# smhassanerfani/nasa-niswan

Hardware: AMD Instinct MI355X
Metric: training samples/sec (90x144x20 grid, seq_len=12) (higher is better)
Workload: dtype bf16; 1 GPU; cfg1-20level; in_channels=62, out_channels=20, seq_len=12, batch_per_gpu=8, global_batch=8, parallelism=dp1, wave=4, overlap_allreduce=False

## Files before the change

nasa-niswan_amd/csrc/wgrad.hip:

```cpp
#include <type_traits>
#include "nint_common.h"

struct WgSrc {
  const char* dG;
  const char* src; long src_img_stride; int src_pix_stride;
  float* partial;
  int CB, JG;
  int nblk;
  int ntiles, tiles_per_split;
  int want_db;
};
struct WgradArgs {
  long dG_img_stride; int dG_pix_stride;
  WgSrc s[2];
  int nparts;
  int NTC, J;
  int TG;
  int k, p, taps;
  int P, Wh;
  int tiles_x, tiles_y;
};

template <int DT> struct WgTile;
template <> struct WgTile<NINT_BF16> { static constexpr int PR = 4, RA = 160; static constexpr int rb(int ntc) { return ntc == 1 ? 32 : 96; } };
template <> struct WgTile<NINT_F32> { static constexpr int PR = 2, RA = 320; static constexpr int rb(int ntc) { return ntc == 1 ? 64 : 192; } };

template <int DT, int JW, int NS, int KS, int NTCT, int KX>
__global__ __launch_bounds__(256, 2) void wgrad_kernel(WgradArgs a) {
  typedef Elem<DT> E;
  typedef WgTile<DT> TT;
  constexpr int PR = TT::PR, RA = TT::RA;
  constexpr int NTN = 4 / NS;
  constexpr int A_UNITS_PIX = 64 * E::ES / 16;

  extern __shared__ __attribute__((aligned(16))) char smem[];
  const int tid = threadIdx.x, lane = tid & 63;
  const int wave = __builtin_amdgcn_readfirstlane(tid >> 6);
  constexpr int p = KS / 2, k = KS;
  constexpr int HWt = 32 + 2 * p, HHt = PR + 2 * p;
  constexpr int RB = TT::rb(NTCT);
  constexpr int b_units_pix = 16 * NTCT * E::ES / 16;
  constexpr int UA_ROW = RA / 16, NA_U = PR * 32 * UA_ROW;
  constexpr int UB_PIX = RB / 16, NB_U = HHt * HWt * UB_PIX, NB_U_PAD = (NB_U + 63) / 64 * 64;
  constexpr int a_bytes = PR * 32 * RA;
  constexpr int b_bytes = NB_U_PAD * 16;
  constexpr int buf_bytes = a_bytes + b_bytes;
  static_assert(NA_U % 64 == 0 && a_bytes % 1024 == 0, "whole DMA pieces");
  constexpr int NI_A = NA_U / 64, NI_B = NB_U_PAD / 64, NI = NI_A + NI_B;

  int by = blockIdx.y, part = 0;
  if (a.nparts == 2) {
    const int per_nb = a.s[0].CB + a.s[1].CB;
    const int nbq = by / per_nb, r = by - nbq * per_nb;
    part = r >= a.s[0].CB ? 1 : 0;
    by = part ? nbq * a.s[1].CB + (r - a.s[0].CB) : nbq * a.s[0].CB + r;
  }
  part = __builtin_amdgcn_readfirstlane(part);
  by = __builtin_amdgcn_readfirstlane(by);
  struct { const char* dG; const char* src; long src_img_stride; int src_pix_stride; float* partial; int CB, JG, nblk, ntiles, tiles_per_split, want_db; } S;
  {
    const WgSrc& T = a.s[part];
    S.dG = T.dG; S.src = T.src; S.src_img_stride = T.src_img_stride; S.src_pix_stride = T.src_pix_stride; S.partial = T.partial;
    S.CB = T.CB; S.JG = T.JG; S.nblk = T.nblk; S.ntiles = T.ntiles; S.tiles_per_split = T.tiles_per_split; S.want_db = T.want_db;
  }
  const int tg = __builtin_amdgcn_readfirstlane(by % a.TG);
  const int bc = __builtin_amdgcn_readfirstlane(by / a.TG);
  const int nb = bc / S.CB, cb = bc % S.CB;
  const int jb = tg * 4 * JW;
  const int t_begin = blockIdx.x * S.tiles_per_split;
  const int t_end = min(S.ntiles, t_begin + S.tiles_per_split);
  const int i0 = (wave % NS) * NTN;
  const int j0 = (wave / NS) * JW;

  f32x4_t acc[NTN][JW];
#pragma unroll
  for (int i = 0; i < NTN; ++i)
#pragma unroll
    for (int j = 0; j < JW; ++j) acc[i][j] = (f32x4_t){0.f, 0.f, 0.f, 0.f};

  const bool do_db = __builtin_amdgcn_readfirstlane((S.want_db && cb == 0 && tg == a.TG - 1 && wave == 3 && NS == 1) ? 1 : 0);

  constexpr int NI_WM = (NI + 1) / 2;
  int p_begin, p_cnt;
  {
    constexpr int CM = (DT == NINT_BF16 ? 16 : 32 * 4) * NTN * PR, CD = 100;
    int nv[4], n16[4], tot = 0, sum_nv = 0;
#pragma unroll
    for (int w = 0; w < 4; ++w) { nv[w] = min(JW, max(0, a.J - jb - (w / NS) * JW)); sum_nv += nv[w]; }
    const int L = (NI * CD + CM * sum_nv) / 4;
#pragma unroll
    for (int w = 0; w < 4; ++w) { n16[w] = max(0, (L - nv[w] * CM) * 16 / CD); tot += n16[w]; }
    int cnt[4], prev = 0, acc16 = 0, excess = 0;
#pragma unroll
    for (int w = 0; w < 4; ++w) {
      acc16 += n16[w];
      const int e = w == 3 ? NI : (tot > 0 ? min(NI, (acc16 * NI + tot / 2) / tot) : (w + 1) * NI / 4);
      cnt[w] = e - prev;
      prev = e;
      if (cnt[w] > NI_WM) { excess += cnt[w] - NI_WM; cnt[w] = NI_WM; }
    }
#pragma unroll
    for (int w = 0; w < 4; ++w) {
      const int take = min(NI_WM - cnt[w], excess);
      cnt[w] += take;
      excess -= take;
    }
    const int s1 = cnt[0], s2 = s1 + cnt[1], s3 = s2 + cnt[2];
    p_begin = __builtin_amdgcn_readfirstlane(wave == 0 ? 0 : (wave == 1 ? s1 : (wave == 2 ? s2 : s3)));
    p_cnt = __builtin_amdgcn_readfirstlane(wave == 0 ? cnt[0] : (wave == 1 ? cnt[1] : (wave == 2 ? cnt[2] : cnt[3])));
  }
  unsigned doff[NI_WM];
#pragma unroll
  for (int i = 0; i < NI_WM; ++i) {
    const int t = p_begin + i;
    unsigned o = 0;
    if (t < NI_A) {
      const int u = t * 64 + lane;
      const int pix = u / UA_ROW, q = u - pix * UA_ROW;
      if (q < A_UNITS_PIX) o = (unsigned)(((pix >> 5) * a.Wh + (pix & 31)) * a.dG_pix_stride + q * 16);
    } else if (t < NI) {
      const int u = (t - NI_A) * 64 + lane;
      const int hp = u / UB_PIX, q = u - hp * UB_PIX;
      const int hy = hp / HWt, hx = hp - hy * HWt;
      if (hp < HHt * HWt && q < b_units_pix) o = (unsigned)((hy * a.Wh + hx) * S.src_pix_stride + q * 16);
    }
    doff[i] = o;
  }
  int ld_tx, ld_ty, ld_img;
  {
    const int r = t_begin / a.tiles_x;
    ld_tx = t_begin - r * a.tiles_x;
    ld_img = r / a.tiles_y;
    ld_ty = r - ld_img * a.tiles_y;
  }
  const char* const ga0 = S.dG + nb * 64 * E::ES;
  const char* const gb0 = S.src + cb * 16 * NTCT * E::ES;

  auto issue_dma = [&](char* buf) {
    const int y0 = ld_ty * PR, x0 = ld_tx * 32;
    const char* ga = ga0 + (long)ld_img * a.dG_img_stride + ((long)(y0 + a.P) * a.Wh + (x0 + a.P)) * a.dG_pix_stride;
    const char* gb = gb0 + (long)ld_img * S.src_img_stride + ((long)(y0 + a.P - p) * a.Wh + (x0 + a.P - p)) * S.src_pix_stride;
#pragma unroll
    for (int i = 0; i < NI_WM; ++i) {
      const int t = p_begin + i;
      if (i < p_cnt) {
        const char* src = (t < NI_A ? ga : gb) + doff[i];
        char* dst = buf + (t < NI_A ? t * 1024 : a_bytes + (t - NI_A) * 1024);
        unsigned keep;
        const unsigned lds_dst = __builtin_amdgcn_readfirstlane((unsigned)(uintptr_t)(__attribute__((address_space(3))) char*)dst);
        asm volatile("s_mov_b32 %0, m0\n\ts_mov_b32 m0, %2\n\ts_nop 0\n\tglobal_load_lds_dwordx4 %1, off\n\ts_mov_b32 m0, %0"
                     : "=&s"(keep) : "v"(src), "s"(lds_dst) : "memory");
      }
    }
    const bool wx = ld_tx + 1 == a.tiles_x;
    const bool wy = wx && (ld_ty + 1 == a.tiles_y);
    ld_tx = wx ? 0 : ld_tx + 1;
    ld_ty = wy ? 0 : (wx ? ld_ty + 1 : ld_ty);
    ld_img += wy ? 1 : 0;
  };

  if (t_begin < t_end) issue_dma(smem);
  asm volatile("s_waitcnt vmcnt(0)" ::: "memory");
  __syncthreads();

  const int g = lane >> 4, i16 = lane & 15;
  int vB[JW];
  int vA;
  const int nvalid = __builtin_amdgcn_readfirstlane(min(JW, max(0, a.J - jb - j0)));
  constexpr int JT = KS * KX * NTCT;
  constexpr int XO = KX == KS ? 0 : p;
  constexpr int NVL = JT % JW == 0 ? JW : JT % JW;
  if constexpr (DT == NINT_BF16) {
    const int q = i16 >> 2, p8 = (i16 & 3) * 8;
    vA = (4 * g + q) * RA + i0 * 32 + p8;
#pragma unroll
    for (int jj = 0; jj < JW; ++jj) {
      const int j = min(jb + j0 + jj, a.J - 1);
      const int tap = j / NTCT, ct = j - tap * NTCT;
      const int tyy = tap / KX, txx = tap - tyy * KX + XO;
      vB[jj] = a_bytes + (tyy * HWt + txx + 4 * g + q) * RB + ct * 32 + p8;
    }
  } else {
    vA = g * RA + (i0 * 16 + i16) * 4;
#pragma unroll
    for (int jj = 0; jj < JW; ++jj) {
      const int j = min(jb + j0 + jj, a.J - 1);
      const int tap = j / NTCT, ct = j - tap * NTCT;
      const int tyy = tap / KX, txx = tap - tyy * KX + XO;
      vB[jj] = a_bytes + (tyy * HWt + txx + g) * RB + (ct * 16 + i16) * 4;
    }
  }
  auto run_tiles = [&](auto nvc, auto dbc) __attribute__((always_inline)) {
    constexpr int NV = decltype(nvc)::value;
    constexpr bool DB = decltype(dbc)::value;
    for (int tile = t_begin; tile < t_end; ++tile) {
      const int cur = (tile - t_begin) & 1;
      const bool more = tile + 1 < t_end;
      if (more) issue_dma(smem + (cur ^ 1) * buf_bytes);
      const char* Ab = smem + cur * buf_bytes + vA;
      const char* Bb[JW];
#pragma unroll
      for (int jj = 0; jj < JW; ++jj) Bb[jj] = smem + cur * buf_bytes + vB[jj];
      if constexpr ((NV > 0 || DB) && DT == NINT_BF16) {
#pragma unroll
        for (int pr = 0; pr < PR; ++pr) {
          auto read_tr = [&](const char* ad, int half) __attribute__((always_inline)) {
            s16x4_t lo = __builtin_amdgcn_ds_read_tr16_b64_v4i16((__attribute__((address_space(3))) s16x4_t*)(ad));
            s16x4_t hi = __builtin_amdgcn_ds_read_tr16_b64_v4i16((__attribute__((address_space(3))) s16x4_t*)(ad + half));
            u32x2_t l2 = __builtin_bit_cast(u32x2_t, lo), h2 = __builtin_bit_cast(u32x2_t, hi);
            return (u32x4_t){l2[0], l2[1], h2[0], h2[1]};
          };
          u32x4_t af[NTN], bf[NV > 0 ? NV : 1];
#pragma unroll
          for (int i = 0; i < NTN; ++i) af[i] = read_tr(Ab + pr * 32 * RA + i * 32, 16 * RA);
#pragma unroll
          for (int jj = 0; jj < NV; ++jj) bf[jj] = read_tr(Bb[jj] + pr * HWt * RB, 16 * RB);
#pragma unroll
          for (int jj = 0; jj < NV; ++jj)
#pragma unroll
            for (int i = 0; i < NTN; ++i) acc[i][jj] = mma_step<NINT_BF16>(af[i], bf[jj], acc[i][jj]);
          if constexpr (DB) {
            const u32x4_t ones = {0x3f803f80u, 0x3f803f80u, 0x3f803f80u, 0x3f803f80u};
#pragma unroll
            for (int i = 0; i < NTN; ++i) acc[i][JW - 1] = mma_step<NINT_BF16>(af[i], ones, acc[i][JW - 1]);
          }
        }
      } else if constexpr (NV > 0 || DB) {
#pragma unroll
        for (int pr = 0; pr < PR; ++pr) {
#pragma unroll
          for (int ks = 0; ks < 2; ++ks) {
#pragma unroll
            for (int m = 0; m < 4; ++m) {
              float af[NTN];
#pragma unroll
              for (int i = 0; i < NTN; ++i)
                af[i] = *(const float*)(Ab + (pr * 32 + ks * 16 + 4 * m) * RA + i * 64);
#pragma unroll
              for (int jj = 0; jj < NV; ++jj) {
                const float bf = *(const float*)(Bb[jj] + (pr * HWt + ks * 16 + 4 * m) * RB);
#pragma unroll
                for (int i = 0; i < NTN; ++i)
                  acc[i][jj] = __builtin_amdgcn_mfma_f32_16x16x4f32(af[i], bf, acc[i][jj], 0, 0, 0);
              }
              if constexpr (DB) {
#pragma unroll
                for (int i = 0; i < NTN; ++i) acc[i][JW - 1] = __builtin_amdgcn_mfma_f32_16x16x4f32(af[i], 1.0f, acc[i][JW - 1], 0, 0, 0);
              }
            }
          }
        }
      }
      asm volatile("s_waitcnt vmcnt(0)" ::: "memory");
      __syncthreads();
    }
  };
  if (do_db) {
    if (NVL < JW && nvalid == NVL) run_tiles(std::integral_constant<int, NVL < JW ? NVL : 0>{}, std::true_type{});
    else run_tiles(std::integral_constant<int, 0>{}, std::true_type{});
  } else {
    if (nvalid == JW) run_tiles(std::integral_constant<int, JW>{}, std::false_type{});
    else if (nvalid == NVL) run_tiles(std::integral_constant<int, NVL>{}, std::false_type{});
    else run_tiles(std::integral_constant<int, 0>{}, std::false_type{});
  }

  float* out = S.partial + ((size_t)blockIdx.x * S.nblk + by) * S.JG * 1024;
#pragma unroll
  for (int jj = 0; jj < JW; ++jj) {
    const int j = j0 + jj;
    if (jb + j < a.J) {
#pragma unroll
      for (int i = 0; i < NTN; ++i)
#pragma unroll
        for (int r = 0; r < 4; ++r)
          out[(size_t)j * 1024 + ((i0 + i) * 16 + 4 * g + r) * 16 + i16] = acc[i][jj][r];
    }
  }
  if (do_db) {
#pragma unroll
    for (int i = 0; i < NTN; ++i)
#pragma unroll
      for (int r = 0; r < 4; ++r)
        out[(size_t)(S.JG - 1) * 1024 + ((i0 + i) * 16 + 4 * g + r) * 16 + i16] = acc[i][JW - 1][r];
  }
}

template <int KS, int NCT> struct WgWide {
  static constexpr int taps = KS * KS;
  static constexpr int HG = KS == 3 ? 1 : (KS == 5 ? 2 : 4);
  static constexpr int JW = (taps + HG - 1) / HG;
  static constexpr int NVL = taps - (HG - 1) * JW;
  static constexpr int JWA = JW + (NVL == JW ? 1 : 0);
  static constexpr int NW = 2 * NCT * HG;
  static constexpr int PR = 4, RA = 288;
  static constexpr int RB = NCT == 4 ? 160 : (NCT == 2 ? 96 : 32);
  static constexpr int p = KS / 2, HWt = 32 + 2 * p, HHt = PR + 2 * p;
  static constexpr int UA_ROW = RA / 16, NA_U = PR * 32 * UA_ROW;
  static constexpr int UB_PIX = RB / 16, NB_U = HHt * HWt * UB_PIX, NB_U_PAD = (NB_U + 63) / 64 * 64;
  static constexpr int a_bytes = PR * 32 * RA, b_bytes = NB_U_PAD * 16, buf_bytes = a_bytes + b_bytes;
  static constexpr int NI_A = NA_U / 64, NI_B = NB_U_PAD / 64, NI = NI_A + NI_B;
  static constexpr int NI_W = (NI + NW - 1) / NW;
  static_assert(NA_U % 64 == 0, "whole DMA pieces");
  static_assert(NW == 8, "eight waves: two per SIMD");
};

template <int KS, int NCT>
__global__ __launch_bounds__(512, 2) void wgrad_wide_kernel(WgradArgs a) {
  typedef WgWide<KS, NCT> G;
  constexpr int PR = G::PR, RA = G::RA, RB = G::RB, HWt = G::HWt, HHt = G::HHt, p = G::p, JW = G::JW, JWA = G::JWA, HG = G::HG;
  constexpr int a_bytes = G::a_bytes, buf_bytes = G::buf_bytes, NI_A = G::NI_A, NI = G::NI, NI_W = G::NI_W;
#ifndef NINT_WG_STREAM
#define NINT_WG_STREAM (JW > 9)
#endif
  constexpr bool STREAM = NINT_WG_STREAM;
  extern __shared__ __attribute__((aligned(16))) char smem[];
  const int tid = threadIdx.x, lane = tid & 63;
  const int wave = __builtin_amdgcn_readfirstlane(tid >> 6);
  const int gh = wave & 1, cgi = wave >> 1, ct = cgi / HG, half = cgi % HG;
  const WgSrc& T = a.s[0];
  const int CBW = T.CB / NCT;
  const int by = blockIdx.y;
  const int nbw = __builtin_amdgcn_readfirstlane(by / CBW), cbw = __builtin_amdgcn_readfirstlane(by % CBW);
  const int t_begin = blockIdx.x * T.tiles_per_split;
  const int t_end = min(T.ntiles, t_begin + T.tiles_per_split);
  const unsigned src_pix_stride = (unsigned)T.src_pix_stride;

  f32x4_t acc[4][JWA];
#pragma unroll
  for (int i = 0; i < 4; ++i)
#pragma unroll
    for (int j = 0; j < JWA; ++j) acc[i][j] = (f32x4_t){0.f, 0.f, 0.f, 0.f};
  const bool do_db = __builtin_amdgcn_readfirstlane((T.want_db && cbw == 0 && ct == 0 && half == HG - 1) ? 1 : 0);

  auto piece_off = [&](int t) __attribute__((always_inline)) {
    unsigned o = 0;
    if (t < NI_A) {
      const unsigned u = (unsigned)(t * 64 + lane);
      const unsigned pix = __umulhi(u, (unsigned)(((1ull << 32) + G::UA_ROW - 1) / G::UA_ROW)), q = u - pix * G::UA_ROW;
      o = q < 16 ? ((pix >> 5) * a.Wh + (pix & 31)) * a.dG_pix_stride + q * 16 : 0u;
    } else {
      const unsigned u = (unsigned)((t - NI_A) * 64 + lane);
      const unsigned hp = __umulhi(u, (unsigned)(((1ull << 32) + G::UB_PIX - 1) / G::UB_PIX)), q = u - hp * G::UB_PIX;
      const unsigned hy = __umulhi(hp, (unsigned)(((1ull << 32) + HWt - 1) / HWt)), hx = hp - hy * HWt;
      o = (hp < (unsigned)(HHt * HWt) && q < 2u * NCT) ? (hy * a.Wh + hx) * src_pix_stride + q * 16 : 0u;
    }
    return o;
  };
  int ld_tx, ld_ty, ld_img;
  {
    const int r = t_begin / a.tiles_x;
    ld_tx = t_begin - r * a.tiles_x;
    ld_img = r / a.tiles_y;
    ld_ty = r - ld_img * a.tiles_y;
  }
  const char* const ga0 = T.dG + nbw * 128 * 2;
  const char* const gb0 = T.src + cbw * 16 * NCT * 2;
  const long src_img_stride = T.src_img_stride;
  auto issue_dma = [&](char* buf) {
    const int y0 = ld_ty * PR, x0 = ld_tx * 32;
    const char* ga = ga0 + (long)ld_img * a.dG_img_stride + ((long)(y0 + a.P) * a.Wh + (x0 + a.P)) * a.dG_pix_stride;
    const char* gb = gb0 + (long)ld_img * src_img_stride + ((long)(y0 + a.P - p) * a.Wh + (x0 + a.P - p)) * src_pix_stride;
#pragma unroll
    for (int i = 0; i < NI_W; ++i) {
      const int t = wave + G::NW * i;
      if (t < NI) {
        const char* src = (t < NI_A ? ga : gb) + piece_off(t);
        char* dst = buf + (t < NI_A ? t * 1024 : a_bytes + (t - NI_A) * 1024);
        unsigned keep;
        const unsigned lds_dst = __builtin_amdgcn_readfirstlane((unsigned)(uintptr_t)(__attribute__((address_space(3))) char*)dst);
        asm volatile("s_mov_b32 %0, m0\n\ts_mov_b32 m0, %2\n\ts_nop 0\n\tglobal_load_lds_dwordx4 %1, off\n\ts_mov_b32 m0, %0"
                     : "=&s"(keep) : "v"(src), "s"(lds_dst) : "memory");
      }
    }
    const bool wx = ld_tx + 1 == a.tiles_x;
    const bool wy = wx && (ld_ty + 1 == a.tiles_y);
    ld_tx = wx ? 0 : ld_tx + 1;
    ld_ty = wy ? 0 : (wx ? ld_ty + 1 : ld_ty);
    ld_img += wy ? 1 : 0;
  };
  if (t_begin < t_end) issue_dma(smem);
  asm volatile("s_waitcnt vmcnt(0)" ::: "memory");
  __syncthreads();

  const int g = lane >> 4, i16 = lane & 15, q4 = i16 >> 2, p8 = (i16 & 3) * 8;
  const int vA = (4 * g + q4) * RA + gh * 128 + p8;
  const int vB = a_bytes + (4 * g + q4) * RB + ct * 32 + p8;

  auto run_tiles = [&](auto tap0c, auto nvc, auto dbc) __attribute__((always_inline)) {
    constexpr int TAP0 = decltype(tap0c)::value, NV = decltype(nvc)::value;
    constexpr bool DB = decltype(dbc)::value;
    for (int tile = t_begin; tile < t_end; ++tile) {
      const int cur = (tile - t_begin) & 1;
      if (tile + 1 < t_end) issue_dma(smem + (cur ^ 1) * buf_bytes);
      const char* Ab = smem + cur * buf_bytes + vA;
      const char* Bb = smem + cur * buf_bytes + vB;
      auto read_tr = [&](const char* ad, int half_off) __attribute__((always_inline)) {
        s16x4_t lo = __builtin_amdgcn_ds_read_tr16_b64_v4i16((__attribute__((address_space(3))) s16x4_t*)(ad));
        s16x4_t hi = __builtin_amdgcn_ds_read_tr16_b64_v4i16((__attribute__((address_space(3))) s16x4_t*)(ad + half_off));
        u32x2_t l2 = __builtin_bit_cast(u32x2_t, lo), h2 = __builtin_bit_cast(u32x2_t, hi);
        return (u32x4_t){l2[0], l2[1], h2[0], h2[1]};
      };
#pragma unroll
      for (int pr = 0; pr < PR; ++pr) {
        u32x4_t af[4];
#pragma unroll
        for (int i = 0; i < 4; ++i) af[i] = read_tr(Ab + pr * 32 * RA + i * 32, 16 * RA);
        auto colptr = [&](int jj) __attribute__((always_inline)) {
          const int tap = TAP0 + jj, tyy = tap / KS, txx = tap - tyy * KS;
          return Bb + (tyy * HWt + txx) * RB + pr * HWt * RB;
        };
        if constexpr (STREAM) {
          u32x4_t bfq[2];
          if constexpr (NV > 0) bfq[0] = read_tr(colptr(0), 16 * RB);
#pragma unroll
          for (int jj = 0; jj < NV; ++jj) {
            if (jj + 1 < NV) bfq[(jj + 1) & 1] = read_tr(colptr(jj + 1), 16 * RB);
#pragma unroll
            for (int i = 0; i < 4; ++i) acc[i][jj] = mma_step<NINT_BF16>(af[i], bfq[jj & 1], acc[i][jj]);
          }
        } else {
#pragma unroll
          for (int jj = 0; jj < NV; ++jj) {
            const u32x4_t bf = read_tr(colptr(jj), 16 * RB);
#pragma unroll
            for (int i = 0; i < 4; ++i) acc[i][jj] = mma_step<NINT_BF16>(af[i], bf, acc[i][jj]);
          }
        }
        if constexpr (DB) {
          const u32x4_t ones = {0x3f803f80u, 0x3f803f80u, 0x3f803f80u, 0x3f803f80u};
#pragma unroll
          for (int i = 0; i < 4; ++i) acc[i][JWA - 1] = mma_step<NINT_BF16>(af[i], ones, acc[i][JWA - 1]);
        }
        if constexpr (STREAM) {
          __builtin_amdgcn_sched_group_barrier(0x100, NV > 0 ? 10 : 8, 0);
#pragma unroll
          for (int jj = 0; jj < NV; ++jj) {
            if (jj + 1 < NV) __builtin_amdgcn_sched_group_barrier(0x100, 2, 0);
            __builtin_amdgcn_sched_group_barrier(0x008, 4, 0);
          }
          if constexpr (DB) __builtin_amdgcn_sched_group_barrier(0x008, 4, 0);
        }
      }
      asm volatile("s_waitcnt vmcnt(0)" ::: "memory");
      __syncthreads();
    }
  };
  auto role = [&](auto hc) __attribute__((always_inline)) {
    constexpr int H_ = decltype(hc)::value;
    constexpr int TAP0 = H_ * JW, NV = H_ == HG - 1 ? G::NVL : JW;
    if (H_ == HG - 1 && do_db) run_tiles(std::integral_constant<int, TAP0>{}, std::integral_constant<int, NV>{}, std::true_type{});
    else run_tiles(std::integral_constant<int, TAP0>{}, std::integral_constant<int, NV>{}, std::false_type{});
  };
  if constexpr (HG == 1) role(std::integral_constant<int, 0>{});
  else if constexpr (HG == 2) { if (half == 0) role(std::integral_constant<int, 0>{}); else role(std::integral_constant<int, 1>{}); }
  else { if (half == 0) role(std::integral_constant<int, 0>{}); else if (half == 1) role(std::integral_constant<int, 1>{});
         else if (half == 2) role(std::integral_constant<int, 2>{}); else role(std::integral_constant<int, 3>{}); }

  const int nb = 2 * nbw + gh, cb = cbw * NCT + ct;
  float* out = T.partial + ((size_t)blockIdx.x * T.nblk + (size_t)nb * T.CB + cb) * T.JG * 1024;
  const int tap0 = half * JW, nv = half == HG - 1 ? G::NVL : JW;
#pragma unroll
  for (int jj = 0; jj < JW; ++jj) {
    if (jj < nv) {
#pragma unroll
      for (int i = 0; i < 4; ++i)
#pragma unroll
        for (int r = 0; r < 4; ++r) out[(size_t)(tap0 + jj) * 1024 + (i * 16 + 4 * g + r) * 16 + i16] = acc[i][jj][r];
    }
  }
  if (do_db) {
#pragma unroll
    for (int i = 0; i < 4; ++i)
#pragma unroll
      for (int r = 0; r < 4; ++r) out[(size_t)(T.JG - 1) * 1024 + (i * 16 + 4 * g + r) * 16 + i16] = acc[i][JWA - 1][r];
  }
}

struct ReduceEntry {
  const float* part; float* dW;
  int Cx, Ch, Ch16, k, NB, CB, NTC, J, splits, is_h, xfold;
  int TG, JG;
  float* db;
  int waves;
  unsigned blk_begin;
};
struct ReduceTable { ReduceEntry e[2 * NINT_MAX_LAYERS]; int n; };

__global__ void wgrad_reduce_kernel(ReduceTable t) {
  __shared__ f32x4_t red[1024];
  int ei = 0;
  for (int q = 1; q < t.n; ++q) ei = blockIdx.x >= t.e[q].blk_begin ? q : ei;
  const ReduceEntry& E = t.e[ei];
  const int Cx = E.Cx, Ch = E.Ch, k = E.k, CB = E.CB, NTC = E.NTC, J = E.J, splits = E.splits, is_h = E.is_h;
  const int TG = E.TG, JG = E.JG;
  const float* __restrict__ part = E.part;
  float* __restrict__ dW = E.dW;
  const int taps = k * k, Ctot = Cx + Ch;
  const size_t slab = (size_t)E.NB * CB * TG * JG * 1024;
  const int lane = threadIdx.x & 63, grp = threadIdx.x >> 6, G = E.waves;
  const size_t i = ((size_t)(blockIdx.x - E.blk_begin) * 64 + lane) * 4;
  f32x4_t s = {0.f, 0.f, 0.f, 0.f};
  if (grp < G) {
#pragma unroll 8
    for (int sp = grp; sp < splits; sp += G) s += __builtin_nontemporal_load((const f32x4_t*)(part + i + (size_t)sp * slab));
  }
  red[threadIdx.x] = s;
  __syncthreads();
  if (grp != 0) return;
  for (int q = 1; q < G; ++q) s += red[q * 64 + lane];
  const int c16 = i & 15, nloc = (i >> 4) & 63;
  size_t r = i >> 10;
  const int jl = r % JG; r /= JG;
  const int tgi = r % TG; r /= TG;
  const int cb = r % CB;
  const int nb = r / CB;
  const int np = nb * 64 + nloc;
  const int ch = (np >> 6) * 16 + (np & 15), gate = (np >> 4) & 3;
  const int JR = JG - (E.db ? 1 : 0);
  if (jl >= JR) {
    if (cb == 0 && tgi == TG - 1 && c16 == 0 && ch < Ch) E.db[gate * Ch + ch] = s[0];
    return;
  }
  const int j = tgi * JR + jl;
  if (j >= J || ch >= Ch) return;
  const int tap0 = j / NTC;
  const int ct = j - tap0 * NTC;
  const int Csrc = is_h ? Ch : Cx;
#pragma unroll
  for (int e = 0; e < 4; ++e) {
    int cc = (cb * NTC + ct) * 16 + c16 + e;
    int tap = tap0;
    if (!is_h && E.xfold) {
      if (cc >= k * Cx) continue;
      tap = tap0 * k + cc / Cx;
      cc = cc % Cx;
    }
    if (cc >= Csrc) continue;
    const int ic = is_h ? Cx + cc : cc;
    dW[(((size_t)(gate * Ch + ch)) * Ctot + ic) * taps + tap] = s[e];
  }
}

struct WgPart { int NTC, J, JW, KX, CB, TG, JG, splits;
                int wide_nct, wcols; };
struct WgPlan {
  WgPart part[2];
  int NB, tiles_x, tiles_y, ntiles;
  size_t off_h, total_floats;
  bool merged;
};

static int wg_wide_nct(const nint_layer* ly, int dtype, int q) {
  if (dtype != NINT_BF16 || ly->wide == 1 || (q == 0 && ly->xfold)) return 0;
  const int nct = ly->k == 3 ? 4 : (ly->k == 5 ? 2 : (ly->k == 7 ? 1 : 0));
  if (!nct || (4 * ly->Ch16) % 128 || (q == 0 ? ly->Cxp : ly->Chp) % (16 * nct)) return 0;
  return nct;
}

#ifndef NINT_WG_MIN_TILES
#define NINT_WG_MIN_TILES 8
#endif
static int wg_plan(const nint_layer* ly, int dtype, int n_cu, int N, const nint_geom* g, WgPlan* pl) {
  if (ly->k != 1 && ly->k != 3 && ly->k != 5 && ly->k != 7) return NINT_E_SHAPE;
  pl->NB = 4 * ly->Ch16 / 64;
  const int PR = dtype == NINT_BF16 ? 4 : 2;
  pl->tiles_x = g ? nint_cdiv(g->W, 32) : 1;
  pl->tiles_y = g ? nint_cdiv(g->H, PR) : 1;
  pl->ntiles = g ? N * pl->tiles_x * pl->tiles_y : (1 << 30);
  if (n_cu <= 0) n_cu = 256;
  size_t floats[2];
  for (int q = 0; q < 2; ++q) {
    WgPart& w = pl->part[q];
    const int Cp = q == 0 ? ly->Cxp : ly->Chp;
    w.wide_nct = wg_wide_nct(ly, dtype, q);
    w.wcols = 0;
    if (w.wide_nct) {
      w.KX = ly->k; w.NTC = 1; w.J = ly->k * ly->k; w.JW = 0; w.TG = 1;
      w.JG = w.J + (q == 0 ? 1 : 0);
      w.CB = Cp / 16;
      w.wcols = (pl->NB / 2) * (w.CB / w.wide_nct);
      int s = nint_cdiv(n_cu, w.wcols);
      if (s > pl->ntiles / NINT_WG_MIN_TILES) s = pl->ntiles / NINT_WG_MIN_TILES;
      if (s < 1) s = 1;
      s = nint_cdiv(pl->ntiles, nint_cdiv(pl->ntiles, s));
      if (s >= 8) s -= s % 8;
      w.splits = s;
      floats[q] = (size_t)w.splits * pl->NB * w.CB * w.JG * 1024;
      continue;
    }
    w.KX = (q == 0 && ly->xfold) ? 1 : ly->k;
    const int taps = ly->k * w.KX;
    w.NTC = (taps * 2 <= 20 && Cp % 32 == 0) ? 2 : 1;
    w.J = taps * w.NTC;
    w.JW = w.J <= 20 ? 5 : 7;
    w.TG = nint_cdiv(w.J, 4 * w.JW);
    w.JG = (w.TG == 1 ? w.J : 4 * w.JW) + (q == 0 ? 1 : 0);
    if (w.TG > 1 && w.J % w.JW) return NINT_E_SHAPE;
    if (q == 0 && w.J - (w.TG - 1) * 4 * w.JW > 3 * w.JW + (w.JW - 1)) return NINT_E_SHAPE;
    const int CW = 16 * w.NTC;
    if (Cp % CW) return NINT_E_SHAPE;
    w.CB = Cp / CW;
#ifndef NINT_WG_MIN_TILES
#define NINT_WG_MIN_TILES 8
#endif
    int s = nint_cdiv(2 * n_cu, pl->NB * w.CB * w.TG);
    if (s > pl->ntiles / NINT_WG_MIN_TILES) s = pl->ntiles / NINT_WG_MIN_TILES;
    if (s < 1) s = 1;
    w.splits = nint_cdiv(pl->ntiles, nint_cdiv(pl->ntiles, s));
    floats[q] = (size_t)w.splits * pl->NB * w.CB * w.TG * w.JG * 1024;
  }
  const WgPart &wx = pl->part[0], &wh = pl->part[1];
  pl->merged = !wx.wide_nct && !wh.wide_nct && wx.NTC == wh.NTC && wx.JW == wh.JW && wx.KX == wh.KX && wx.TG == 1 && wh.TG == 1 && pl->NB * (wx.CB + wh.CB) <= 8;
  if (pl->merged) {
    int s = nint_cdiv(2 * n_cu, pl->NB * (wx.CB + wh.CB));
    if (s > pl->ntiles / NINT_WG_MIN_TILES) s = pl->ntiles / NINT_WG_MIN_TILES;
    if (s < 1) s = 1;
    s = nint_cdiv(pl->ntiles, nint_cdiv(pl->ntiles, s));
    if (s >= 8) s -= s % 8;
    for (int q = 0; q < 2; ++q) {
      WgPart& w = pl->part[q];
      w.splits = s;
      floats[q] = (size_t)w.splits * pl->NB * w.CB * w.TG * w.JG * 1024;
    }
  }
  pl->off_h = floats[0];
  pl->total_floats = floats[0] + floats[1];
  return NINT_OK;
}

extern "C" size_t nint_wgrad_workspace_bytes(const nint_layer* ly, int dtype, int n_cu) {
  if (!ly) return 0;
  WgPlan pl;
  if (wg_plan(ly, dtype, n_cu, 1, nullptr, &pl) != NINT_OK) return 0;
  return pl.total_floats * sizeof(float);
}

template <int DT, int JW, int KS, int NTCT, int KX>
static int launch_wgrad(WgradArgs& a, int splits, int nblk, hipStream_t st) {
  typedef WgTile<DT> TT;
  const int p = a.p;
  const int a_bytes = TT::PR * 32 * TT::RA;
  const int b_bytes = nint_round_up((TT::PR + 2 * p) * (32 + 2 * p) * TT::rb(a.NTC), 1024);
  const size_t lds = 2 * (size_t)(a_bytes + b_bytes);
  if (lds > 160 * 1024) return NINT_E_LDS;
  if (a.k != KS || a.NTC != NTCT || a.J != KS * KX * NTCT) return NINT_E_ARG;
  auto kern = wgrad_kernel<DT, JW, 1, KS, NTCT, KX>;
  if (lds > 64 * 1024)
    NINT_CHECK_HIP(hipFuncSetAttribute((const void*)kern, hipFuncAttributeMaxDynamicSharedMemorySize, (int)lds));
  hipLaunchKernelGGL(kern, dim3(splits, nblk), dim3(256), lds, st, a);
  NINT_LAUNCH_CHECK();
  return NINT_OK;
}

template <int KS, int NCT>
static int launch_wgrad_wide(WgradArgs& a, int splits, int cols, hipStream_t st) {
  typedef WgWide<KS, NCT> G;
  const size_t lds = 2 * (size_t)G::buf_bytes;
  if (lds > 160 * 1024) return NINT_E_LDS;
  auto kern = wgrad_wide_kernel<KS, NCT>;
  NINT_CHECK_HIP(hipFuncSetAttribute((const void*)kern, hipFuncAttributeMaxDynamicSharedMemorySize, (int)lds));
  hipLaunchKernelGGL(kern, dim3(splits, cols), dim3(512), lds, st, a);
  NINT_LAUNCH_CHECK();
  return NINT_OK;
}

template <int DT>
static int dispatch_wgrad(WgradArgs& a, const WgPart& w, int nblk, hipStream_t st) {
  const int key = a.k * 1000 + w.NTC * 100 + w.JW * 10 + w.KX;
  switch (key) {
    case 5 * 1000 + 1 * 100 + 7 * 10 + 5: return launch_wgrad<DT, 7, 5, 1, 5>(a, w.splits, nblk, st);
    case 3 * 1000 + 2 * 100 + 5 * 10 + 3: return launch_wgrad<DT, 5, 3, 2, 3>(a, w.splits, nblk, st);
    case 3 * 1000 + 1 * 100 + 5 * 10 + 3: return launch_wgrad<DT, 5, 3, 1, 3>(a, w.splits, nblk, st);
    case 1 * 1000 + 2 * 100 + 5 * 10 + 1: return launch_wgrad<DT, 5, 1, 2, 1>(a, w.splits, nblk, st);
    case 1 * 1000 + 1 * 100 + 5 * 10 + 1: return launch_wgrad<DT, 5, 1, 1, 1>(a, w.splits, nblk, st);
    case 5 * 1000 + 2 * 100 + 5 * 10 + 1: return launch_wgrad<DT, 5, 5, 2, 1>(a, w.splits, nblk, st);
    case 5 * 1000 + 1 * 100 + 5 * 10 + 1: return launch_wgrad<DT, 5, 5, 1, 1>(a, w.splits, nblk, st);
    case 3 * 1000 + 2 * 100 + 5 * 10 + 1: return launch_wgrad<DT, 5, 3, 2, 1>(a, w.splits, nblk, st);
    case 3 * 1000 + 1 * 100 + 5 * 10 + 1: return launch_wgrad<DT, 5, 3, 1, 1>(a, w.splits, nblk, st);
    case 7 * 1000 + 1 * 100 + 7 * 10 + 7: return launch_wgrad<DT, 7, 7, 1, 7>(a, w.splits, nblk, st);
    case 7 * 1000 + 2 * 100 + 5 * 10 + 1: return launch_wgrad<DT, 5, 7, 2, 1>(a, w.splits, nblk, st);
    case 7 * 1000 + 1 * 100 + 5 * 10 + 1: return launch_wgrad<DT, 5, 7, 1, 1>(a, w.splits, nblk, st);
    default: return NINT_E_SHAPE;
  }
}

int nint_internal_conv_wgrad_multi(const WgJob* jobs, int njobs, const nint_geom* g, int dtype, float* partial,
                                   size_t partial_bytes, int n_cu, void* stream, Probe* probe) {
  if (!jobs || njobs < 1 || njobs > NINT_MAX_LAYERS || !g || !partial) return NINT_E_ARG;
  if (dtype != NINT_F32 && dtype != NINT_BF16) return NINT_E_ARG;
  const int es = dtype == NINT_BF16 ? 2 : 4;
  hipStream_t st = (hipStream_t)stream;
  ReduceTable rt = {};
  size_t off = 0;
  unsigned blk = 0;
  int red_threads = 256;
  for (int q = 0; q < njobs; ++q) {
    const WgJob& jb = jobs[q];
    const nint_layer* ly = jb.ly;
    if (!ly || !jb.dG || !jb.x_slab || !jb.h_slab || !jb.dW || !jb.db || jb.N <= 0) return NINT_E_ARG;
    if (jb.h_skip < 0 || jb.h_skip > jb.N) return NINT_E_ARG;
    WgPlan pl;
    int rc = wg_plan(ly, dtype, n_cu, jb.N, g, &pl);
    if (rc != NINT_OK) return rc;
    if ((off + pl.total_floats) * sizeof(float) > partial_bytes) return NINT_E_ARG;
    float* base = partial + off;
    off += (pl.total_floats + 63) / 64 * 64;
    const int Gc = 4 * ly->Ch16;
    WgradArgs a = {};
    a.dG_pix_stride = Gc * es;
    a.dG_img_stride = (long)g->Hh * g->Wh * a.dG_pix_stride;
    a.k = ly->k; a.p = ly->k / 2;
    a.P = g->P; a.Wh = g->Wh;
    a.tiles_x = pl.tiles_x; a.tiles_y = pl.tiles_y;
    if (probe) probe->stamp(NINT_PROBE_WGRAD, q, 0, 0);
    for (int part = 0; part < 2; ++part) {
      const WgPart& w = pl.part[part];
      WgSrc& S = a.s[pl.merged ? part : 0];
      const int skip = part == 1 ? jb.h_skip : 0;
      S.dG = (const char*)jb.dG + (size_t)skip * a.dG_img_stride;
      const int Cp = part == 0 ? ly->Cxp : ly->Chp;
      S.src_pix_stride = Cp * es;
      S.src_img_stride = (long)g->Hh * g->Wh * S.src_pix_stride;
      S.src = (const char*)(part == 0 ? jb.x_slab : jb.h_slab) + (size_t)skip * S.src_img_stride;
      S.partial = base + (part == 0 ? 0 : pl.off_h);
      S.CB = w.CB; S.JG = w.JG;
      S.nblk = pl.NB * w.CB * w.TG;
      S.want_db = part == 0 ? 1 : 0;
      S.ntiles = (jb.N - skip) * pl.tiles_x * pl.tiles_y;
      S.tiles_per_split = S.ntiles > 0 ? nint_cdiv(S.ntiles, w.splits) : 1;
      a.NTC = w.NTC; a.J = w.J; a.TG = w.TG;
      a.taps = ly->k * w.KX;
      if (w.wide_nct) {
        a.nparts = 1;
        rc = ly->k == 3 ? launch_wgrad_wide<3, 4>(a, w.splits, w.wcols, st)
           : (ly->k == 5 ? launch_wgrad_wide<5, 2>(a, w.splits, w.wcols, st) : launch_wgrad_wide<7, 1>(a, w.splits, w.wcols, st));
        if (rc != NINT_OK) return rc;
      } else if (!pl.merged || part == 1) {
        a.nparts = pl.merged ? 2 : 1;
        const int nblk = pl.merged ? a.s[0].nblk + a.s[1].nblk : S.nblk;
        rc = dtype == NINT_BF16 ? dispatch_wgrad<NINT_BF16>(a, w, nblk, st) : dispatch_wgrad<NINT_F32>(a, w, nblk, st);
        if (rc != NINT_OK) return rc;
      }
      ReduceEntry& E = rt.e[rt.n++];
      E.part = S.partial; E.dW = jb.dW; E.db = part == 0 ? jb.db : nullptr;
      E.Cx = ly->Cx; E.Ch = ly->Ch; E.Ch16 = ly->Ch16; E.k = ly->k; E.NB = pl.NB; E.CB = w.CB; E.NTC = w.NTC; E.J = w.J;
      E.splits = w.splits; E.is_h = part; E.xfold = ly->xfold; E.TG = w.TG; E.JG = w.JG;
      E.blk_begin = blk;
      blk += (unsigned)((size_t)pl.NB * w.CB * w.TG * w.JG * 1024 / 256);
      E.waves = 4;
      if (E.waves * 64 > red_threads) red_threads = E.waves * 64;
    }
    if (probe) probe->stamp(NINT_PROBE_WGRAD, q, 0, 1);
  }
  if (probe) probe->stamp(NINT_PROBE_FOLD, 0, 0, 0);
  hipLaunchKernelGGL(wgrad_reduce_kernel, dim3(blk), dim3(red_threads), 0, st, rt);
  NINT_LAUNCH_CHECK();
  if (probe) probe->stamp(NINT_PROBE_FOLD, 0, 0, 1);
  return NINT_OK;
}

extern "C" int nint_conv_wgrad(const nint_layer* ly, const nint_geom* g, int dtype, int N, const void* dG,
                               const void* x_slab, const void* h_slab, float* dW, float* db, float* partial,
                               size_t partial_bytes, int n_cu, void* stream) {
  const WgJob jb = {ly, N, dG, x_slab, h_slab, dW, db, 0};
  return nint_internal_conv_wgrad_multi(&jb, 1, g, dtype, partial, partial_bytes, n_cu, stream);
}
```

Baseline: 1079 samples/s.

## Merge x/h wide wgrad launches, stagger DMA issue across waves, rebalance wave roles

```diff
diff --git a/nasa-niswan_amd/csrc/wgrad.hip b/nasa-niswan_amd/csrc/wgrad.hip
--- a/nasa-niswan_amd/csrc/wgrad.hip
+++ b/nasa-niswan_amd/csrc/wgrad.hip
@@ -312,14 +312,41 @@
 #ifndef NINT_WG_STREAM
 #define NINT_WG_STREAM (JW > 9)
 #endif
+#ifndef NINT_WG_STAG
+#define NINT_WG_STAG 1
+#endif
+#ifndef NINT_WG_STAG_SPREAD
+#define NINT_WG_STAG_SPREAD 0
+#endif
+#ifndef NINT_WG_PRIO
+#define NINT_WG_PRIO 0
+#endif
+#ifndef NINT_WG_BALANCE
+#define NINT_WG_BALANCE 1
+#endif
   constexpr bool STREAM = NINT_WG_STREAM;
   extern __shared__ __attribute__((aligned(16))) char smem[];
   const int tid = threadIdx.x, lane = tid & 63;
   const int wave = __builtin_amdgcn_readfirstlane(tid >> 6);
-  const int gh = wave & 1, cgi = wave >> 1, ct = cgi / HG, half = cgi % HG;
-  const WgSrc& T = a.s[0];
+  __builtin_assume(wave >= 0 && wave < G::NW);
+  const int gh = wave & 1, cgi = wave >> 1;
+  const int ct = HG == 2 && NINT_WG_BALANCE ? wave >> 2 : cgi / HG;
+  const int half = HG == 2 && NINT_WG_BALANCE ? (cgi ^ (wave >> 2)) & 1 : cgi % HG;
+  int by = blockIdx.y, part = 0;
+  if (a.nparts == 2) {
+    const int cols_x = a.s[0].nblk / (2 * NCT);
+    part = by >= cols_x ? 1 : 0;
+    by -= part ? cols_x : 0;
+  }
+  part = __builtin_amdgcn_readfirstlane(part);
+  by = __builtin_amdgcn_readfirstlane(by);
+  struct { const char* dG; const char* src; long src_img_stride; int src_pix_stride; float* partial; int CB, JG, nblk, ntiles, tiles_per_split, want_db; } T;
+  {
+    const WgSrc& Q = a.s[part];
+    T.dG = Q.dG; T.src = Q.src; T.src_img_stride = Q.src_img_stride; T.src_pix_stride = Q.src_pix_stride; T.partial = Q.partial;
+    T.CB = Q.CB; T.JG = Q.JG; T.nblk = Q.nblk; T.ntiles = Q.ntiles; T.tiles_per_split = Q.tiles_per_split; T.want_db = Q.want_db;
+  }
   const int CBW = T.CB / NCT;
-  const int by = blockIdx.y;
   const int nbw = __builtin_amdgcn_readfirstlane(by / CBW), cbw = __builtin_amdgcn_readfirstlane(by % CBW);
   const int t_begin = blockIdx.x * T.tiles_per_split;
   const int t_end = min(T.ntiles, t_begin + T.tiles_per_split);
@@ -332,7 +359,7 @@
     for (int j = 0; j < JWA; ++j) acc[i][j] = (f32x4_t){0.f, 0.f, 0.f, 0.f};
   const bool do_db = __builtin_amdgcn_readfirstlane((T.want_db && cbw == 0 && ct == 0 && half == HG - 1) ? 1 : 0);
 
-  auto piece_off = [&](int t) __attribute__((always_inline)) {
+  auto piece_off = [&](int t, unsigned lane) __attribute__((always_inline)) {
     unsigned o = 0;
     if (t < NI_A) {
       const unsigned u = (unsigned)(t * 64 + lane);
@@ -356,42 +383,85 @@
   const char* const ga0 = T.dG + nbw * 128 * 2;
   const char* const gb0 = T.src + cbw * 16 * NCT * 2;
   const long src_img_stride = T.src_img_stride;
-  auto issue_dma = [&](char* buf) {
+  auto issue_dma = [&](char* buf, int i_lo, int i_hi, bool last) __attribute__((always_inline)) {
     const int y0 = ld_ty * PR, x0 = ld_tx * 32;
     const char* ga = ga0 + (long)ld_img * a.dG_img_stride + ((long)(y0 + a.P) * a.Wh + (x0 + a.P)) * a.dG_pix_stride;
     const char* gb = gb0 + (long)ld_img * src_img_stride + ((long)(y0 + a.P - p) * a.Wh + (x0 + a.P - p)) * src_pix_stride;
+    unsigned ln = (unsigned)lane;
+    asm volatile("" : "+v"(ln));
 #pragma unroll
     for (int i = 0; i < NI_W; ++i) {
-      const int t = wave + G::NW * i;
-      if (t < NI) {
-        const char* src = (t < NI_A ? ga : gb) + piece_off(t);
+      const int t = min(wave + G::NW * i, NI - 1);
+      if (i >= i_lo && i < i_hi) {
+        const char* base = t < NI_A ? ga : gb;
+        const unsigned off = piece_off(t, ln);
         char* dst = buf + (t < NI_A ? t * 1024 : a_bytes + (t - NI_A) * 1024);
         unsigned keep;
         const unsigned lds_dst = __builtin_amdgcn_readfirstlane((unsigned)(uintptr_t)(__attribute__((address_space(3))) char*)dst);
-        asm volatile("s_mov_b32 %0, m0\n\ts_mov_b32 m0, %2\n\ts_nop 0\n\tglobal_load_lds_dwordx4 %1, off\n\ts_mov_b32 m0, %0"
-                     : "=&s"(keep) : "v"(src), "s"(lds_dst) : "memory");
+        asm volatile("s_mov_b32 %0, m0\n\ts_mov_b32 m0, %2\n\ts_nop 0\n\tglobal_load_lds_dwordx4 %1, %3\n\ts_mov_b32 m0, %0"
+                     : "=&s"(keep) : "v"(off), "s"(lds_dst), "s"(base) : "memory");
       }
     }
-    const bool wx = ld_tx + 1 == a.tiles_x;
-    const bool wy = wx && (ld_ty + 1 == a.tiles_y);
-    ld_tx = wx ? 0 : ld_tx + 1;
-    ld_ty = wy ? 0 : (wx ? ld_ty + 1 : ld_ty);
-    ld_img += wy ? 1 : 0;
+    if (last) {
+      const bool wx = ld_tx + 1 == a.tiles_x;
+      const bool wy = wx && (ld_ty + 1 == a.tiles_y);
+      ld_tx = wx ? 0 : ld_tx + 1;
+      ld_ty = wy ? 0 : (wx ? ld_ty + 1 : ld_ty);
+      ld_img += wy ? 1 : 0;
+    }
   };
-  if (t_begin < t_end) issue_dma(smem);
+  if (t_begin < t_end) issue_dma(smem, 0, NI_W, true);
   asm volatile("s_waitcnt vmcnt(0)" ::: "memory");
   __syncthreads();
+  constexpr int STAG = NINT_WG_STAG;
+  constexpr bool SPREAD = NINT_WG_STAG_SPREAD;
+  const bool late = __builtin_amdgcn_readfirstlane(wave >= 4 ? 1 : 0);
+#if NINT_WG_PRIO
+  if (late) __builtin_amdgcn_s_setprio(1);
+#endif
 
   const int g = lane >> 4, i16 = lane & 15, q4 = i16 >> 2, p8 = (i16 & 3) * 8;
   const int vA = (4 * g + q4) * RA + gh * 128 + p8;
   const int vB = a_bytes + (4 * g + q4) * RB + ct * 32 + p8;
 
-  auto run_tiles = [&](auto tap0c, auto nvc, auto dbc) __attribute__((always_inline)) {
+  auto flush = [&]() __attribute__((always_inline)) {
+    const int nb = 2 * nbw + gh, cb = cbw * NCT + ct;
+    float* out = T.partial + ((size_t)blockIdx.x * T.nblk + (size_t)nb * T.CB + cb) * T.JG * 1024;
+    const int tap0 = half * JW, nv = half == HG - 1 ? G::NVL : JW;
+#pragma unroll
+    for (int jj = 0; jj < JW; ++jj) {
+      if (jj < nv) {
+#pragma unroll
+        for (int i = 0; i < 4; ++i)
+#pragma unroll
+          for (int r = 0; r < 4; ++r) out[(size_t)(tap0 + jj) * 1024 + (i * 16 + 4 * g + r) * 16 + i16] = acc[i][jj][r];
+      }
+    }
+    if (do_db) {
+#pragma unroll
+      for (int i = 0; i < 4; ++i)
+#pragma unroll
+        for (int r = 0; r < 4; ++r) out[(size_t)(T.JG - 1) * 1024 + (i * 16 + 4 * g + r) * 16 + i16] = acc[i][JWA - 1][r];
+    }
+  };
+  auto run_tiles = [&](auto tap0c, auto nvc, auto dbc, auto latec) __attribute__((always_inline)) {
     constexpr int TAP0 = decltype(tap0c)::value, NV = decltype(nvc)::value;
-    constexpr bool DB = decltype(dbc)::value;
+    constexpr bool DB = decltype(dbc)::value, LATE = decltype(latec)::value;
     for (int tile = t_begin; tile < t_end; ++tile) {
       const int cur = (tile - t_begin) & 1;
-      if (tile + 1 < t_end) issue_dma(smem + (cur ^ 1) * buf_bytes);
+      const bool more = tile + 1 < t_end;
+      char* const nbuf = smem + (cur ^ 1) * buf_bytes;
+      auto stage = [&](int pr) __attribute__((always_inline)) {
+#ifndef NINT_WG_ABLATE_DMA
+        if constexpr (SPREAD) {
+          constexpr int H1 = (NI_W + 1) / 2, R0 = LATE ? 2 : 0;
+          if (pr == R0 && more) issue_dma(nbuf, 0, H1, false);
+          if (pr == R0 + 1 && more) issue_dma(nbuf, H1, NI_W, true);
+        } else {
+          if (pr == (LATE ? STAG : 0) && more) issue_dma(nbuf, 0, NI_W, true);
+        }
+#endif
+      };
       const char* Ab = smem + cur * buf_bytes + vA;
       const char* Bb = smem + cur * buf_bytes + vB;
       auto read_tr = [&](const char* ad, int half_off) __attribute__((always_inline)) {
@@ -402,6 +472,7 @@
       };
 #pragma unroll
       for (int pr = 0; pr < PR; ++pr) {
+        stage(pr);
         u32x4_t af[4];
 #pragma unroll
         for (int i = 0; i < 4; ++i) af[i] = read_tr(Ab + pr * 32 * RA + i * 32, 16 * RA);
@@ -444,36 +515,21 @@
       asm volatile("s_waitcnt vmcnt(0)" ::: "memory");
       __syncthreads();
     }
+    flush();
   };
   auto role = [&](auto hc) __attribute__((always_inline)) {
     constexpr int H_ = decltype(hc)::value;
     constexpr int TAP0 = H_ * JW, NV = H_ == HG - 1 ? G::NVL : JW;
-    if (H_ == HG - 1 && do_db) run_tiles(std::integral_constant<int, TAP0>{}, std::integral_constant<int, NV>{}, std::true_type{});
-    else run_tiles(std::integral_constant<int, TAP0>{}, std::integral_constant<int, NV>{}, std::false_type{});
+    auto pos = [&](auto dbc) __attribute__((always_inline)) {
+      if ((STAG > 0 || SPREAD) && late) run_tiles(std::integral_constant<int, TAP0>{}, std::integral_constant<int, NV>{}, dbc, std::true_type{});
+      else run_tiles(std::integral_constant<int, TAP0>{}, std::integral_constant<int, NV>{}, dbc, std::false_type{});
+    };
+    if (H_ == HG - 1 && do_db) pos(std::true_type{}); else pos(std::false_type{});
   };
   if constexpr (HG == 1) role(std::integral_constant<int, 0>{});
   else if constexpr (HG == 2) { if (half == 0) role(std::integral_constant<int, 0>{}); else role(std::integral_constant<int, 1>{}); }
   else { if (half == 0) role(std::integral_constant<int, 0>{}); else if (half == 1) role(std::integral_constant<int, 1>{});
          else if (half == 2) role(std::integral_constant<int, 2>{}); else role(std::integral_constant<int, 3>{}); }
-
-  const int nb = 2 * nbw + gh, cb = cbw * NCT + ct;
-  float* out = T.partial + ((size_t)blockIdx.x * T.nblk + (size_t)nb * T.CB + cb) * T.JG * 1024;
-  const int tap0 = half * JW, nv = half == HG - 1 ? G::NVL : JW;
-#pragma unroll
-  for (int jj = 0; jj < JW; ++jj) {
-    if (jj < nv) {
-#pragma unroll
-      for (int i = 0; i < 4; ++i)
-#pragma unroll
-        for (int r = 0; r < 4; ++r) out[(size_t)(tap0 + jj) * 1024 + (i * 16 + 4 * g + r) * 16 + i16] = acc[i][jj][r];
-    }
-  }
-  if (do_db) {
-#pragma unroll
-    for (int i = 0; i < 4; ++i)
-#pragma unroll
-      for (int r = 0; r < 4; ++r) out[(size_t)(T.JG - 1) * 1024 + (i * 16 + 4 * g + r) * 16 + i16] = acc[i][JWA - 1][r];
-  }
 }
 
 struct ReduceEntry {
@@ -547,6 +603,7 @@
   WgPart part[2];
   int NB, tiles_x, tiles_y, ntiles;
   size_t off_h, total_floats;
+  bool wide_merged;
   bool merged;
 };
 
@@ -559,6 +616,9 @@
 
 #ifndef NINT_WG_MIN_TILES
 #define NINT_WG_MIN_TILES 8
+#endif
+#ifndef NINT_WG_MERGE_WIDE
+#define NINT_WG_MERGE_WIDE 1
 #endif
 static int wg_plan(const nint_layer* ly, int dtype, int n_cu, int N, const nint_geom* g, WgPlan* pl) {
   if (ly->k != 1 && ly->k != 3 && ly->k != 5 && ly->k != 7) return NINT_E_SHAPE;
@@ -611,6 +671,7 @@
   }
   const WgPart &wx = pl->part[0], &wh = pl->part[1];
   pl->merged = !wx.wide_nct && !wh.wide_nct && wx.NTC == wh.NTC && wx.JW == wh.JW && wx.KX == wh.KX && wx.TG == 1 && wh.TG == 1 && pl->NB * (wx.CB + wh.CB) <= 8;
+  pl->wide_merged = NINT_WG_MERGE_WIDE && wx.wide_nct && wx.wide_nct == wh.wide_nct && wx.splits == wh.splits;
   if (pl->merged) {
     int s = nint_cdiv(2 * n_cu, pl->NB * (wx.CB + wh.CB));
     if (s > pl->ntiles / NINT_WG_MIN_TILES) s = pl->ntiles / NINT_WG_MIN_TILES;
@@ -715,7 +776,7 @@
     if (probe) probe->stamp(NINT_PROBE_WGRAD, q, 0, 0);
     for (int part = 0; part < 2; ++part) {
       const WgPart& w = pl.part[part];
-      WgSrc& S = a.s[pl.merged ? part : 0];
+      WgSrc& S = a.s[(pl.merged || pl.wide_merged) ? part : 0];
       const int skip = part == 1 ? jb.h_skip : 0;
       S.dG = (const char*)jb.dG + (size_t)skip * a.dG_img_stride;
       const int Cp = part == 0 ? ly->Cxp : ly->Chp;
@@ -731,10 +792,13 @@
       a.NTC = w.NTC; a.J = w.J; a.TG = w.TG;
       a.taps = ly->k * w.KX;
       if (w.wide_nct) {
-        a.nparts = 1;
-        rc = ly->k == 3 ? launch_wgrad_wide<3, 4>(a, w.splits, w.wcols, st)
-           : (ly->k == 5 ? launch_wgrad_wide<5, 2>(a, w.splits, w.wcols, st) : launch_wgrad_wide<7, 1>(a, w.splits, w.wcols, st));
-        if (rc != NINT_OK) return rc;
+        if (!pl.wide_merged || part == 1) {
+          a.nparts = pl.wide_merged ? 2 : 1;
+          const int cols = pl.wide_merged ? pl.part[0].wcols + w.wcols : w.wcols;
+          rc = ly->k == 3 ? launch_wgrad_wide<3, 4>(a, w.splits, cols, st)
+             : (ly->k == 5 ? launch_wgrad_wide<5, 2>(a, w.splits, cols, st) : launch_wgrad_wide<7, 1>(a, w.splits, cols, st));
+          if (rc != NINT_OK) return rc;
+        }
       } else if (!pl.merged || part == 1) {
         a.nparts = pl.merged ? 2 : 1;
         const int nblk = pl.merged ? a.s[0].nblk + a.s[1].nblk : S.nblk;
```

New measurement: 1042 samples/s. 0.966x the previous value.
